# lrjconan/LanczosNetwork

Measured on AMD Instinct MI355X. Metric: molecules/sec LanczosNet forward, QM8 batch=1024, higher is better.
Workload: dtype f32; 1 GPU; QM8 LanczosNet batch=1024/GPU, N<=32 dense L (tile N=26), K=20, fp32, 7x128 layers, 1xMI355X per rank; step = [pack L + batch plan + Lanczos + tridiagonal eigensolver (Ritz pairs)] (one launch) + spectral gains + fused forward; global_batch=1024, parallelism=dp1 (batch shards, async score all-gather per step)

## Files before the change

lanczosnet_amd/csrc/gains_body.hpp:

```cpp
#pragma once
#include "common.hpp"

namespace lnz_gains {

constexpr int HID = 128;
constexpr int HT = HID / 32;
constexpr int SMAX = 16;
constexpr int OFF_W0 = 0;
constexpr int OFF_B0 = OFF_W0 + HT * 8 * 64;
constexpr int OFF_B2 = OFF_B0 + HT * 1024;
constexpr int OFF_B4 = OFF_B2 + HT * 1024;
constexpr int OFF_B6 = OFF_B4 + HT * 1024;
constexpr int OFF_W2 = OFF_B6 + 1024;
constexpr int OFF_W4 = OFF_W2 + HT * 16 * 256;
constexpr int OFF_W6 = OFF_W4 + HT * 16 * 256;
#ifndef LNZ_GAINS_RING
#define LNZ_GAINS_RING 8
#endif
#ifndef LNZ_GAINS_DIST
#define LNZ_GAINS_DIST (LNZ_GAINS_RING - 2)
#endif
constexpr int RING = LNZ_GAINS_RING;
constexpr int PACK_SIZE = OFF_W6 + 16 * 256 + RING * 256;
constexpr int NSTEP = 2 * HT * 16 + 16;

struct DistArr {
  int32_t v[SMAX];
};

__device__ inline float powi(float x, int p) {
  double base = (double)x, acc = 1.0;
  int e = p < 0 ? -p : p;
  while (e) {
    if (e & 1) acc *= base;
    base *= base;
    e >>= 1;
  }
  return (float)(p < 0 ? 1.0 / acc : acc);
}

__device__ inline f32x16 load_bias_frag(const float* __restrict__ bp, int lane) {
  const float4* p = reinterpret_cast<const float4*>(bp) + lane * 4;
  f32x16 acc;
#pragma unroll
  for (int g = 0; g < 4; ++g) {
    float4 v = p[g];
    acc[4 * g + 0] = v.x;
    acc[4 * g + 1] = v.y;
    acc[4 * g + 2] = v.z;
    acc[4 * g + 3] = v.w;
  }
  return acc;
}

__device__ inline f32x16 relu_bias16(f32x16 v, f32x16 b) {
#pragma unroll
  for (int i = 0; i < 16; ++i) v[i] = fmaxf(v[i] + b[i], 0.0f);
  return v;
}

template <int F0, int RT>
__device__ inline void dense_tile(const float4* __restrict__ wstream, float4 (&ring)[RING],
                                  const f32x16 (&Hin)[RT][HT], f32x16 (&res)[RT]) {
  f32x16 acc[RT], acc1[RT];
#pragma unroll
  for (int t = 0; t < RT; ++t) {
    acc[t] = lnz::splat16(0.0f);
    acc1[t] = lnz::splat16(0.0f);
  }
#pragma unroll
  for (int q = 0; q < 16; ++q) {
    constexpr int D = LNZ_GAINS_DIST;
#ifdef LNZ_GAINS_PROBE_NOLOAD
    ring[(F0 + q + D) % RING] = make_float4(0.5f, 0.25f, 0.125f, 1.0f);
#else
    ring[(F0 + q + D) % RING] = wstream[(F0 + q + D) * 64];
#endif
    __builtin_amdgcn_sched_barrier(0);
    const float4 a = ring[(F0 + q) % RING];
    const int ti = q >> 2, g = q & 3;
#pragma unroll
    for (int t = 0; t < RT; ++t) acc[t] = lnz::mfma32(a.x, Hin[t][ti][4 * g + 0], acc[t]);
#pragma unroll
    for (int t = 0; t < RT; ++t) acc1[t] = lnz::mfma32(a.y, Hin[t][ti][4 * g + 1], acc1[t]);
#pragma unroll
    for (int t = 0; t < RT; ++t) acc[t] = lnz::mfma32(a.z, Hin[t][ti][4 * g + 2], acc[t]);
#pragma unroll
    for (int t = 0; t < RT; ++t) acc1[t] = lnz::mfma32(a.w, Hin[t][ti][4 * g + 3], acc1[t]);
    __builtin_amdgcn_sched_barrier(0);
  }
#pragma unroll
  for (int t = 0; t < RT; ++t) {
#pragma unroll
    for (int i = 0; i < 16; ++i) res[t][i] = acc[t][i] + acc1[t][i];
  }
}

template <int RT>
__device__ __forceinline__ void gains_mlp_tiles(const float* __restrict__ D, const int (&row)[RT],
                                                const bool (&valid)[RT], const int l,
                                                const int lane, int B, int K, const DistArr& dist,
                                                int S, const float* __restrict__ mlp_pack,
                                                float* __restrict__ G) {
  const int hh = lane >> 5;
  const float* pk = mlp_pack + (int64_t)l * PACK_SIZE;
#ifdef LNZ_GAINS_PROBE_STAGGER
  for (int i = 0; i < (int)((blockIdx.x & (LNZ_GAINS_PROBE_STAGGER_N - 1)) * LNZ_GAINS_PROBE_STAGGER); ++i)
    __builtin_amdgcn_s_sleep(16);
#endif

  const float4* __restrict__ wstream = reinterpret_cast<const float4*>(pk + OFF_W2) + lane;
  float4 ring[RING];
#pragma unroll
  for (int f = 0; f < LNZ_GAINS_DIST; ++f) ring[f] = wstream[f * 64];

  const int steps0 = S < 8 ? S : 8;
  f32x16 h1[RT][HT], h2[RT][HT];
  {
    float w0[HT][8];
#pragma unroll
    for (int ot = 0; ot < HT; ++ot) {
#pragma unroll
      for (int t = 0; t < 8; ++t) w0[ot][t] = pk[OFF_W0 + (ot * 8 + t) * 64 + lane];
    }
#pragma unroll
    for (int rt = 0; rt < RT; ++rt) {
      const float dval = valid[rt] ? D[row[rt]] : 0.0f;
      float feat[8];
#pragma unroll
      for (int t = 0; t < 8; ++t) {
#ifdef LNZ_GAINS_PROBE_NOPOW
        float lo = t < S ? dval : 0.0f;
        float hi = (8 + t) < S ? dval : 0.0f;
#else
        float lo = t < S ? powi(dval, dist.v[t]) : 0.0f;
        float hi = (8 + t) < S ? powi(dval, dist.v[8 + t]) : 0.0f;
#endif
        feat[t] = hh ? hi : lo;
      }
#pragma unroll
      for (int ot = 0; ot < HT; ++ot) {
        f32x16 acc = lnz::splat16(0.0f);
#pragma unroll
        for (int t = 0; t < 8; ++t) {
          if (t < steps0) acc = lnz::mfma32(w0[ot][t], feat[t], acc);
        }
        h1[rt][ot] = relu_bias16(acc, load_bias_frag(pk + OFF_B0 + ot * 1024, lane));
      }
    }
  }
  f32x16 res[RT];
#define LNZ_DENSE(F0, IN, OUT, OT, BOFF)                                   \
  {                                                                        \
    const f32x16 bb = load_bias_frag(pk + (BOFF), lane);                   \
    dense_tile<F0, RT>(wstream, ring, IN, res);                            \
    _Pragma("unroll") for (int rt = 0; rt < RT; ++rt) OUT[rt][OT] = relu_bias16(res[rt], bb); \
  }
  LNZ_DENSE(0, h1, h2, 0, OFF_B2 + 0 * 1024)
  LNZ_DENSE(16, h1, h2, 1, OFF_B2 + 1 * 1024)
  LNZ_DENSE(32, h1, h2, 2, OFF_B2 + 2 * 1024)
  LNZ_DENSE(48, h1, h2, 3, OFF_B2 + 3 * 1024)
  LNZ_DENSE(64, h2, h1, 0, OFF_B4 + 0 * 1024)
  LNZ_DENSE(80, h2, h1, 1, OFF_B4 + 1 * 1024)
  LNZ_DENSE(96, h2, h1, 2, OFF_B4 + 2 * 1024)
  LNZ_DENSE(112, h2, h1, 3, OFF_B4 + 3 * 1024)
#undef LNZ_DENSE
  {
    const f32x16 b6 = load_bias_frag(pk + OFF_B6, lane);
    dense_tile<128, RT>(wstream, ring, h1, res);
#pragma unroll
    for (int rt = 0; rt < RT; ++rt) {
      if (valid[rt]) {
        const int b = row[rt] / K, k = row[rt] - b * K;
        float* Gb = G + (((int64_t)l * B + b) * S) * K + k;
#pragma unroll
        for (int r = 0; r < 16; ++r) {
          int sidx = lnz::cd_row(r, hh);
          if (sidx < S) Gb[(int64_t)sidx * K] = res[rt][r] + b6[r];
        }
      }
    }
  }
}

__device__ __forceinline__ void gains_mlp_tile(const float* __restrict__ D, const int row,
                                               const bool valid, const int l, const int lane,
                                               int B, int K, const DistArr& dist, int S,
                                               const float* __restrict__ mlp_pack,
                                               float* __restrict__ G) {
  const int rows1[1] = {row};
  const bool valid1[1] = {valid};
  gains_mlp_tiles<1>(D, rows1, valid1, l, lane, B, K, dist, S, mlp_pack, G);
}

}
```

lanczosnet_amd/csrc/lanczos_ritz.hip:

```cpp
#include "common.hpp"
#include "prep.hpp"
#include "gains_body.hpp"

namespace {

constexpr double kBreakdownTol = 1e-8;
constexpr double kEps = 2.220446049250313e-16;

struct Ritz32Smem {
  static constexpr int LD = 34;
  double* Qt;
  double* za;
  double* zb;
  double* ca;
  double* cb;
  double* dd;
  double* Dw;
  double2* de;
  int* perm;
  float* sgn;
  int NR;
  __device__ __forceinline__ double& dw(int hh, int i, int rr) const { return Dw[(hh * NR + i) * 32 + rr]; }
};

// ... 729 lines not shown
      const bool on = r < kk;
      double v[16];
      load16(&sm.Qt[(on ? sm.perm[r] : 0) * LD + 16 * h], v);
      double best = 0.0;
      float sg = 1.0f;
#pragma unroll
      for (int x = 0; x < 16; ++x) {
        const double av = fabs(v[x]);
        const bool take = av > best;
        sg = take ? (v[x] < 0 ? -1.0f : 1.0f) : sg;
        best = take ? av : best;
      }
      double best_up;
      const double best_lo = both_halves(best, best_up);
      int sg_up;
      const int sg_lo = both_halves(__float_as_int(sg), sg_up);
      if (on && h == 0) sm.sgn[r] = __int_as_float(best_up > best_lo ? sg_up : sg_lo);
    }
    __syncthreads();
  }

  for (int k = lane; k < K; k += 64) D[(int64_t)b * K + k] = k < kk ? (float)sm.dd[sm.perm[k]] : 0.0f;
  float* Vb = V + (int64_t)b * N * K;
  if (K <= 64) {
    const int rpp = 64 / K;
    const int rr0 = lane / K, k = lane - rr0 * K;
    const bool lane_on = rr0 < rpp, col_on = lane_on && k < kk;
    const double* col = &sm.Qt[(col_on ? sm.perm[k] : 0) * LD];
    const float sg = col_on ? sm.sgn[k] : 0.0f;
#pragma unroll 4
    for (int r0 = 0; r0 < N; r0 += rpp) {
      const int rr = r0 + rr0;
      if (lane_on && rr < N) Vb[rr * K + k] = (col_on && rr < n) ? sg * (float)col[rr] : 0.0f;
    }
  } else {
    const int dq = 64 / K, dr = 64 - dq * K;
    int rr = lane / K, k = lane - rr * K;
    for (int idx = lane; idx < N * K; idx += 64) {
      float v = 0.0f;
      if (rr < n && k < kk) v = sm.sgn[k] * (float)sm.Qt[sm.perm[k] * LD + rr];
      Vb[idx] = v;
      rr += dq;
      k += dr;
      if (k >= K) k -= K, ++rr;
    }
  }
  if (info && lane == 0) info[b] = nrestart;
#ifdef LNZ_PROFILE_PHASES
  __syncthreads();
  if (lane == 0) {
    long long tp3 = clock64();
    D[(int64_t)b * K + 0] = (float)(tp1 - tp0);
    D[(int64_t)b * K + 1] = (float)(tp2 - tp1);
    D[(int64_t)b * K + 2] = (float)(tp3 - tp2);
    D[(int64_t)b * K + 3] = (float)n;
    D[(int64_t)b * K + 4] = (float)(tsx[1] - tsx[0]);
    D[(int64_t)b * K + 5] = (float)(tsx[2] - tsx[1]);
    D[(int64_t)b * K + 6] = (float)(tsx[3] - tsx[2]);
    D[(int64_t)b * K + 7] = (float)(tsx[4] - tsx[1]);
    D[(int64_t)b * K + 8] = (float)(tsx[5] - tsx[4]);
  }
#endif
}

#ifdef LNZ_RITZ_VGPR160
#define LNZ_RITZ32_ATTR __attribute__((amdgpu_num_vgpr(80)))
#else
#define LNZ_RITZ32_ATTR
#endif
__global__ __launch_bounds__(64) LNZ_RITZ32_ATTR void lanczos_ritz32_kernel(
    const float* __restrict__ A, int64_t sb, int64_t sr, int64_t sc,
    const int32_t* __restrict__ n_nodes, int N, int K, float* __restrict__ D,
    float* __restrict__ V, int32_t* __restrict__ info) {
  extern __shared__ __attribute__((aligned(16))) unsigned char ubuf[];
  lanczos_ritz32_body(A, sb, sr, sc, n_nodes, N, K, D, V, info, blockIdx.x, threadIdx.x,
                      ritz32_view(ubuf, N));
}

__global__ __launch_bounds__(256) __attribute__((amdgpu_waves_per_eu(3)))
void prepare_batch_union_kernel(
    const float* __restrict__ L, int64_t sb, int64_t sr, int64_t sc, int64_t sch, int N, int C,
    float4* __restrict__ Lp, const uint8_t* __restrict__ mask, int B, int n_cu, int allow_pairs,
    int wg_cap, int32_t* __restrict__ plan, int32_t* __restrict__ n_wg, int K,
    int32_t* __restrict__ gain_rows, int32_t* __restrict__ n_gain_rows,
    const int32_t* __restrict__ n_nodes, float* __restrict__ D, float* __restrict__ V,
    int32_t* __restrict__ info, uint32_t* __restrict__ ident, int32_t* __restrict__ strips,
    int32_t* __restrict__ n_strips) {
  extern __shared__ __attribute__((aligned(16))) unsigned char ubuf[];
  const int blk = blockIdx.x;
#ifdef LNZ_PREP_X_NOPLAN
  if (blk < 2) return;
#endif
#ifdef LNZ_PREP_X_EMPTYPACK
  if (blk > B + 1) return;
#endif
  if (blk < 2) {
    __builtin_amdgcn_s_setprio(3);
    if (blk == 0)
      plan_tiles_body(mask, B, N, n_cu, allow_pairs, wg_cap, plan, n_wg, K, gain_rows, n_gain_rows);
    else if (strips)
      plan_strips_body(mask, B, N, n_cu, strips, n_strips, ubuf);
  } else if (blk <= B + 1) {
    if (threadIdx.x >= 64) return;
    lanczos_ritz32_body(L, sb, sr, sc, n_nodes, N, K, D, V, info, blk - 2, threadIdx.x,
                        ritz32_view(ubuf, N));
  } else {
    pack_laplacian_body(L, sb, sr, sc, sch, N, C, Lp, reinterpret_cast<float*>(ubuf), blk - 2 - B,
                        ident);
  }
}

static size_t prep_lds_bytes(int N, int C) {
  size_t lds = (size_t)N * N * C * sizeof(float);
  lds = lds > ritz32_lds_bytes(N) ? lds : ritz32_lds_bytes(N);
  return lds > (size_t)kStripScratch ? lds : (size_t)kStripScratch;
}

__global__ __launch_bounds__(256, 2) void prepare_batch_gains_kernel(
    const float* __restrict__ L, int64_t sb, int64_t sr, int64_t sc, int64_t sch, int N, int C,
    float4* __restrict__ Lp, const uint8_t* __restrict__ mask, int B, int n_cu, int allow_pairs,
    int wg_cap, int32_t* __restrict__ plan, int32_t* __restrict__ n_wg, int K,
    int32_t* __restrict__ gain_rows, int32_t* __restrict__ n_gain_rows,
    const int32_t* __restrict__ n_nodes, float* __restrict__ D, float* __restrict__ V,
    lnz_gains::DistArr dist, int S, int num_layer,
    const float* __restrict__ mlp_pack, float* __restrict__ G, uint32_t* __restrict__ ident,
    int n_cons, const float* __restrict__ Dg, const int32_t* __restrict__ rows_g,
    const int32_t* __restrict__ n_rows_g, int Bg, int32_t* __restrict__ strips,
    int32_t* __restrict__ n_strips) {
  extern __shared__ __attribute__((aligned(16))) unsigned char ubuf[];
  const Ritz32Smem sm = ritz32_view(ubuf, N);
  float* tile = reinterpret_cast<float*>(ubuf);
  const int blk = blockIdx.x;
  if (blk < 2) {
    __builtin_amdgcn_s_setprio(3);
    if (blk == 0)
      plan_tiles_body(mask, B, N, n_cu, allow_pairs, wg_cap, plan, n_wg, K, gain_rows, n_gain_rows);
    else if (strips)
      plan_strips_body(mask, B, N, n_cu, strips, n_strips, ubuf);
  } else if (blk <= B + 1) {
    if (threadIdx.x >= 64) return;
    __builtin_amdgcn_s_setprio(3);
    lanczos_ritz32_body(L, sb, sr, sc, n_nodes, N, K, D, V, nullptr, blk - 2, threadIdx.x, sm);
  } else {
    const int p = blk - B - 2;
    if (p >= n_cons) {
      pack_laplacian_body(L, sb, sr, sc, sch, N, C, Lp, tile, p - n_cons, ident);
      return;
    }
    const int lane = threadIdx.x & 63;
    const int gw = p * 4 + (threadIdx.x >> 6);
    const int t = gw / num_layer, l = gw - t * num_layer;
    const int R = *n_rows_g;
    if (32 * t >= R) return;
    const int idx = 32 * t + (lane & 31);
    const bool valid = idx < R;
    const int row = valid ? rows_g[idx] : 0;
    lnz_gains::gains_mlp_tile(Dg, row, valid, l, lane, Bg, K, dist, S, mlp_pack, G);
  }
}

}

extern "C" int lnz_prepare_batch(const float* L, int64_t stride_b, int64_t stride_r,
                                 int64_t stride_c, int64_t stride_ch, int B, int N, int C,
                                 float* Lp, const uint8_t* mask, const int32_t* n_nodes, int n_cu,
                                 int allow_pairs, int32_t* plan, int32_t* n_wg, int K,
                                 int32_t* gain_rows, int32_t* n_gain_rows, float* D, float* V,
                                 int32_t* info, uint32_t* ident, int32_t* strips,
                                 int32_t* n_strips, lnz_stream_t stream) {
  LNZ_REQUIRE(L && mask && n_nodes && plan && n_wg && D && V && B > 0 && C > 0 &&
                  C <= LNZ_MAX_CHANNELS && n_cu > 0 && K > 0,
              LNZ_EINVAL, "lnz_prepare_batch: bad arguments (B=%d C=%d K=%d)", B, C, K);
  LNZ_REQUIRE(Lp || !ident, LNZ_EINVAL, "lnz_prepare_batch: ident needs Lp (the pack writes both)");
  LNZ_REQUIRE(N > 0 && N <= LNZ_TILE, LNZ_ENOTSUP, "lnz_prepare_batch: N=%d > %d", N, LNZ_TILE);
  LNZ_REQUIRE(!gain_rows || n_gain_rows, LNZ_EINVAL, "lnz_prepare_batch: gain_rows needs n_gain_rows");
  const size_t tile = (size_t)N * N * C * sizeof(float);
  LNZ_REQUIRE(tile <= 40 * 1024, LNZ_ENOTSUP,
              "lnz_prepare_batch: N*N*C*4 = %zu B exceeds the 40 KiB staging tile", tile);
  LNZ_REQUIRE(!strips || n_strips, LNZ_EINVAL, "lnz_prepare_batch: strips need n_strips");
  hipLaunchKernelGGL(prepare_batch_union_kernel, dim3(Lp ? 2 * B + 2 : B + 2), dim3(256),
                     Lp ? prep_lds_bytes(N, C) : prep_lds_bytes(N, 0),
                     (hipStream_t)stream, L, stride_b, stride_r, stride_c, stride_ch, N, C,
                     (float4*)Lp, mask, B, n_cu, allow_pairs, lnz_plan_wg_cap(B, n_cu), plan, n_wg,
                     K, gain_rows, n_gain_rows, n_nodes, D, V, info, ident, strips, n_strips);
  return lnz::check_launch("lnz_prepare_batch");
}

extern "C" int lnz_prepare_batch_prev_gains(
    const float* L, int64_t stride_b, int64_t stride_r, int64_t stride_c, int64_t stride_ch, int B,
    int N, int C, float* Lp, const uint8_t* mask, const int32_t* n_nodes, int n_cu, int allow_pairs,
    int32_t* plan, int32_t* n_wg, int K, int32_t* gain_rows, int32_t* n_gain_rows, float* D,
    float* V, uint32_t* ident, const float* D_prev, int B_prev, const int32_t* rows_prev,
    const int32_t* n_rows_prev, const int32_t* dist_host, int S, int num_layer,
    const float* mlp_pack, float* G_prev, int32_t* strips, int32_t* n_strips,
    lnz_stream_t stream) {
  LNZ_REQUIRE(L && Lp && mask && n_nodes && plan && n_wg && gain_rows && n_gain_rows && D && V &&
                  D_prev && rows_prev && n_rows_prev && dist_host && mlp_pack && G_prev && B > 0 &&
                  B_prev > 0 && C > 0 && C <= LNZ_MAX_CHANNELS && n_cu > 0 && K > 0 && num_layer > 0,
              LNZ_EINVAL, "lnz_prepare_batch_prev_gains: bad arguments (B=%d C=%d K=%d)", B, C, K);
  LNZ_REQUIRE(N > 0 && N <= LNZ_TILE, LNZ_ENOTSUP, "lnz_prepare_batch_prev_gains: N=%d > %d", N,
              LNZ_TILE);
  LNZ_REQUIRE(S >= 1 && S <= lnz_gains::SMAX, LNZ_ENOTSUP, "lnz_prepare_batch_prev_gains: S=%d", S);
  const size_t tile = (size_t)N * N * C * sizeof(float);
  LNZ_REQUIRE(tile <= 40 * 1024, LNZ_ENOTSUP,
              "lnz_prepare_batch_prev_gains: N*N*C*4 = %zu B exceeds the 40 KiB staging tile", tile);
  lnz_gains::DistArr dist;
  for (int i = 0; i < lnz_gains::SMAX; ++i) dist.v[i] = i < S ? dist_host[i] : 0;
  const int64_t tiles = ((int64_t)B_prev * K + 31) / 32;
  const int64_t n_cons = (tiles * num_layer + 3) / 4;
  const int64_t grid = 2 * (int64_t)B + 2 + n_cons;
  LNZ_REQUIRE(grid < (1ll << 31), LNZ_ENOTSUP, "lnz_prepare_batch_prev_gains: batch too large");
  hipLaunchKernelGGL(prepare_batch_gains_kernel, dim3((unsigned)grid), dim3(256),
                     prep_lds_bytes(N, C), (hipStream_t)stream, L, stride_b, stride_r, stride_c, stride_ch, N, C,
                     (float4*)Lp, mask, B, n_cu, allow_pairs, lnz_plan_wg_cap(B, n_cu), plan, n_wg,
                     K, gain_rows, n_gain_rows, n_nodes, D, V, dist, S, num_layer, mlp_pack, G_prev,
                     ident, (int)n_cons, D_prev, rows_prev, n_rows_prev, B_prev,
                     (strips && n_strips) ? strips : nullptr, n_strips);
  return lnz::check_launch("lnz_prepare_batch_prev_gains");
}

int lnz_launch_ritz_wg(const float* A, int64_t stride_b, int64_t stride_r, int64_t stride_c,
                       const int32_t* n_nodes, int B, int N, int K, float* D, float* V,
                       int32_t* info, void* workspace, int64_t workspace_bytes, int flags,
                       hipStream_t s);

extern "C" int lnz_lanczos_ritz(const float* A, int64_t stride_b, int64_t stride_r,
                                int64_t stride_c, const int32_t* n_nodes, int B, int N, int K,
                                float* D, float* V, int32_t* info, lnz_stream_t stream) {
  LNZ_REQUIRE(A && n_nodes && D && V && B > 0 && N > 0 && K > 0, LNZ_EINVAL,
              "lnz_lanczos_ritz: bad arguments (B=%d N=%d K=%d)", B, N, K);
  hipStream_t s = (hipStream_t)stream;
  if (N > 32)
    return lnz_launch_ritz_wg(A, stride_b, stride_r, stride_c, n_nodes, B, N, K, D, V, info, nullptr,
                              0, 0, s);
  hipLaunchKernelGGL(lanczos_ritz32_kernel, dim3(B), dim3(64), ritz32_lds_bytes(N), s, A, stride_b,
                     stride_r, stride_c, n_nodes, N, K, D, V, info);
  return lnz::check_launch("lnz_lanczos_ritz");
}

namespace {
__global__ __launch_bounds__(64) void tridiag_eigh_kernel(const double* __restrict__ diag,
                                                          const double* __restrict__ offd, int M,
                                                          double* __restrict__ R,
                                                          double* __restrict__ Bm) {
  constexpr int NMAX = 64, LD = NMAX + 2;
  __shared__ double Qt[NMAX * LD];
  __shared__ double dd[NMAX], ee[NMAX];
  __shared__ int perm[NMAX];
  const int b = blockIdx.x, lane = threadIdx.x, n = M;
  for (int idx = lane; idx < NMAX * LD; idx += 64) {
    int i = idx / LD, r = idx - i * LD;
    Qt[idx] = (i == r) ? 1.0 : 0.0;
  }
  dd[lane] = lane < n ? diag[(int64_t)b * M + lane] : 0.0;
  ee[lane] = lane < n - 1 ? offd[(int64_t)b * (M - 1) + lane] : 0.0;
  __syncthreads();
  double f = 0.0, tst1 = 0.0;
  for (int l = 0; l < n; ++l) {
    tst1 = fmax(tst1, fabs(dd[l]) + fabs(ee[l]));
    int m = l;
    while (m < n - 1 && fabs(ee[m]) > kEps * tst1) ++m;
    if (m > l) {
      int iter = 0;
      double el;
      do {
        ++iter;
        double g = dd[l];
        el = ee[l];
        double p = (dd[l + 1] - g) / (2.0 * el);
        double rr = sqrt(p * p + 1.0);
        if (p < 0) rr = -rr;
        const double dl = el / (p + rr), dl1 = el * (p + rr), hh = g - dl;
        __syncthreads();
        if (lane == 0) {
          dd[l] = dl;
          dd[l + 1] = dl1;
        }
        if (lane >= l + 2 && lane < n) dd[lane] -= hh;
        __syncthreads();
        f += hh;
        p = dd[m];
        double c = 1.0, c2 = 1.0, c3 = 1.0, s = 0.0, s2 = 0.0;
        const double el1 = ee[l + 1];
        double carry = Qt[m * LD + lane];
        for (int i = m - 1; i >= l; --i) {
          c3 = c2;
          c2 = c;
          s2 = s;
          const double ei = ee[i], di = dd[i];
          g = c * ei;
          const double hp = c * p;
          const double tt = fma(p, p, ei * ei);
          const double rinv = rsqrt(tt), rad = tt * rinv;
          const double e_next = s * rad;
          s = ei * rinv;
          c = p * rinv;
          p = c * di - s * g;
          const double d_next = hp + s * (c * g + s * di);
          ee[i + 1] = e_next;
          dd[i + 1] = d_next;
          const double z0 = Qt[i * LD + lane];
          Qt[(i + 1) * LD + lane] = s * z0 + c * carry;
          carry = c * z0 - s * carry;
        }
        Qt[l * LD + lane] = carry;
        p = -s * s2 * c3 * el1 * ee[l] / dl1;
        el = s * p;
        __syncthreads();
        if (lane == 0) {
          ee[l] = el;
// ... 37 lines not shown
```

lanczosnet_amd/csrc/spectral_gains.hip:

```cpp
#include "common.hpp"
#include "gains_body.hpp"
#include "split_pack.hpp"
#include <stdlib.h>

namespace {

using namespace lnz_gains;

__global__ void pack_w0_kernel(const float* __restrict__ W0, int S, float* __restrict__ out) {
  int idx = blockIdx.x * blockDim.x + threadIdx.x;
  if (idx >= HT * 8 * 64) return;
  int lane = idx & 63, t = (idx >> 6) & 7, ot = idx >> 9;
  int f = 8 * (lane >> 5) + t;
  out[idx] = f < S ? W0[(32 * ot + (lane & 31)) * S + f] : 0.0f;
}

struct SplitRide {
  const float4* pack;
  float4* dst;
  int64_t n4;
  int main_x;
};
__device__ __forceinline__ bool ride_along(const SplitRide& r, const int lane) {
  if (!r.pack || (int)blockIdx.x < r.main_x) return false;
  const int64_t chunk = (int64_t)(blockIdx.x - r.main_x) * gridDim.y + blockIdx.y;
  if (chunk * lnz::kSplitChunk < r.n4) lnz::split_pack_chunk<64>(r.pack, r.dst, r.n4, chunk, lane);
  return true;
}

__global__ __launch_bounds__(64) void spectral_gains_mlp_kernel(
    const float* __restrict__ D, int R, int B, int K, DistArr dist, int S,
    const float* __restrict__ mlp_pack, const int32_t* __restrict__ rows,
    const int32_t* __restrict__ n_rows, float* __restrict__ G, const SplitRide ride) {
  const int lane = threadIdx.x;
  if (ride_along(ride, lane)) return;
  if (rows) R = *n_rows;
  if ((int)blockIdx.x * 32 >= R) return;
  const int idx = blockIdx.x * 32 + (lane & 31);
  const bool valid = idx < R;
  const int row = valid ? (rows ? rows[idx] : idx) : 0;
  gains_mlp_tile(D, row, valid, blockIdx.y, lane, B, K, dist, S, mlp_pack, G);
}

__global__ __launch_bounds__(64) void spectral_gains_mlp2_kernel(
    const float* __restrict__ D, int R, int B, int K, DistArr dist, int S,
    const float* __restrict__ mlp_pack, const int32_t* __restrict__ rows,
    const int32_t* __restrict__ n_rows, float* __restrict__ G, const SplitRide ride) {
  const int lane = threadIdx.x;
  if (ride_along(ride, lane)) return;
  if (rows) R = *n_rows;
  if ((int)blockIdx.x * 64 >= R) return;
  int row[2];
  bool valid[2];
#pragma unroll
  for (int t = 0; t < 2; ++t) {
    const int idx = blockIdx.x * 64 + 32 * t + (lane & 31);
    valid[t] = idx < R;
    row[t] = valid[t] ? (rows ? rows[idx] : idx) : 0;
  }
  gains_mlp_tiles<2>(D, row, valid, blockIdx.y, lane, B, K, dist, S, mlp_pack, G);
}

__global__ void spectral_gains_pow_kernel(const float* __restrict__ D, int B, int K, DistArr dist,
                                          int S, int num_layer, float* __restrict__ G) {
  int64_t idx = (int64_t)blockIdx.x * blockDim.x + threadIdx.x;
  int64_t total = (int64_t)num_layer * B * S * K;
  if (idx >= total) return;
  int k = (int)(idx % K);
  int s = (int)((idx / K) % S);
  int b = (int)((idx / ((int64_t)K * S)) % B);
  G[idx] = powi(D[(int64_t)b * K + k], dist.v[s]);
}

}

extern "C" int64_t lnz_spectral_mlp_pack_size(int S) {
  (void)S;
  return PACK_SIZE;
}

extern "C" int lnz_pack_spectral_mlp(const float* W0, const float* b0, const float* W2,
                                     const float* b2, const float* W4, const float* b4,
                                     const float* W6, const float* b6, int S, float* pack,
                                     lnz_stream_t stream) {
  LNZ_REQUIRE(W0 && b0 && W2 && b2 && W4 && b4 && W6 && b6 && pack, LNZ_EINVAL,
              "lnz_pack_spectral_mlp: null pointer");
  LNZ_REQUIRE(S >= 1 && S <= SMAX, LNZ_ENOTSUP, "lnz_pack_spectral_mlp: S=%d not in 1..%d", S,
              SMAX);
  hipLaunchKernelGGL(pack_w0_kernel, dim3((HT * 8 * 64 + 255) / 256), dim3(256), 0,
                     (hipStream_t)stream, W0, S, pack + OFF_W0);
  int rc = lnz::check_launch("lnz_pack_spectral_mlp(W0)");
  if (rc) return rc;
  if ((rc = lnz_pack_bias_rows(b0, HID, pack + OFF_B0, stream))) return rc;
  if ((rc = lnz_pack_rows_k8(W2, HID, HID, HID, pack + OFF_W2, stream))) return rc;
  if ((rc = lnz_pack_bias_rows(b2, HID, pack + OFF_B2, stream))) return rc;
  if ((rc = lnz_pack_rows_k8(W4, HID, HID, HID, pack + OFF_W4, stream))) return rc;
  if ((rc = lnz_pack_bias_rows(b4, HID, pack + OFF_B4, stream))) return rc;
  if ((rc = lnz_pack_rows_k8(W6, S, HID, HID, pack + OFF_W6, stream))) return rc;
  if ((rc = lnz_pack_bias_rows(b6, S, pack + OFF_B6, stream))) return rc;
  return LNZ_OK;
}

struct MlpLayerPtrs {
  const float* p[16][8];
};

__device__ inline float rows_k8_elem(const float* __restrict__ W, int rows, int cols, int ld,
                                     int Q, int f) {
  const int idx4 = f >> 2, u = f & 3;
  const int lane = idx4 & 63, q = (idx4 >> 6) % Q, rt = (idx4 >> 6) / Q;
  const int row = 32 * rt + (lane & 31), col = 8 * q + 4 * (lane >> 5) + u;
  return (row < rows && col < cols) ? W[(int64_t)row * ld + col] : 0.0f;
}

__device__ inline float bias_rows_elem(const float* __restrict__ b, int rows, int f) {
  const int r = f & 15, lane = (f >> 4) & 63, rt = f >> 10;
  const int row = 32 * rt + lnz::cd_row(r, lane >> 5);
  return row < rows ? b[row] : 0.0f;
}

__global__ void pack_spectral_mlp_layers_kernel(MlpLayerPtrs ptrs, int S, float* __restrict__ pack) {
  const int f = blockIdx.x * blockDim.x + threadIdx.x;
  if (f >= PACK_SIZE) return;
  const int l = blockIdx.y;
  const float* const* pl = ptrs.p[l];
  float v = 0.0f;
  if (f < OFF_B0) {
    const int lane = f & 63, t = (f >> 6) & 7, ot = f >> 9;
    const int feat = 8 * (lane >> 5) + t;
    v = feat < S ? pl[0][(32 * ot + (lane & 31)) * S + feat] : 0.0f;
  } else if (f < OFF_B2) {
    v = bias_rows_elem(pl[1], HID, f - OFF_B0);
  } else if (f < OFF_B4) {
    v = bias_rows_elem(pl[3], HID, f - OFF_B2);
  } else if (f < OFF_B6) {
    v = bias_rows_elem(pl[5], HID, f - OFF_B4);
  } else if (f < OFF_W2) {
    v = bias_rows_elem(pl[7], S, f - OFF_B6);
  } else if (f < OFF_W4) {
    v = rows_k8_elem(pl[2], HID, HID, HID, HID / 8, f - OFF_W2);
  } else if (f < OFF_W6) {
    v = rows_k8_elem(pl[4], HID, HID, HID, HID / 8, f - OFF_W4);
  } else if (f < OFF_W6 + 16 * 256) {
    v = rows_k8_elem(pl[6], S, HID, HID, HID / 8, f - OFF_W6);
  }
  pack[(int64_t)l * PACK_SIZE + f] = v;
}

extern "C" int lnz_pack_spectral_mlp_layers(const float* const* ptrs, int num_layer, int S,
                                            float* pack, lnz_stream_t stream) {
  LNZ_REQUIRE(ptrs && pack && num_layer >= 1 && num_layer <= 16, LNZ_EINVAL,
              "lnz_pack_spectral_mlp_layers: bad arguments (L=%d)", num_layer);
  LNZ_REQUIRE(S >= 1 && S <= SMAX, LNZ_ENOTSUP, "lnz_pack_spectral_mlp_layers: S=%d not in 1..%d",
              S, SMAX);
  MlpLayerPtrs mp;
  for (int l = 0; l < 16; ++l)
    for (int i = 0; i < 8; ++i) {
      mp.p[l][i] = l < num_layer ? ptrs[l * 8 + i] : nullptr;
      LNZ_REQUIRE(l >= num_layer || mp.p[l][i], LNZ_EINVAL,
                  "lnz_pack_spectral_mlp_layers: null pointer (layer %d, tensor %d)", l, i);
    }
  hipLaunchKernelGGL(pack_spectral_mlp_layers_kernel, dim3((PACK_SIZE + 255) / 256, num_layer),
                     dim3(256), 0, (hipStream_t)stream, mp, S, pack);
  return lnz::check_launch("lnz_pack_spectral_mlp_layers");
}

extern "C" int lnz_spectral_gains_rows_split_to(const float* D, int B, int K, const int32_t* dist_host,
                                                int S, int num_layer, int kind, const float* mlp_pack,
                                                const int32_t* rows, const int32_t* n_rows, float* G,
                                                const float* Lp_split, uint16_t* Lp_dst, int64_t lp_floats,
                                                lnz_stream_t stream) {
  LNZ_REQUIRE(!Lp_split == !Lp_dst, LNZ_EINVAL, "lnz_spectral_gains_rows_split_to: pack and destination come together");
  LNZ_REQUIRE(!rows || n_rows, LNZ_EINVAL, "lnz_spectral_gains_rows: rows without n_rows");
  LNZ_REQUIRE(!Lp_split || (kind == 0 && lp_floats > 0 && lp_floats % 4 == 0), LNZ_EINVAL,
              "lnz_spectral_gains_rows_split: the pack rides along with the MLP launch only (kind 0), "
              "lp_floats a positive multiple of 4");
  LNZ_REQUIRE(D && dist_host && G && B > 0 && K > 0 && num_layer > 0, LNZ_EINVAL,
              "lnz_spectral_gains: bad arguments (B=%d K=%d L=%d)", B, K, num_layer);
  LNZ_REQUIRE(S >= 1 && S <= SMAX, LNZ_ENOTSUP, "lnz_spectral_gains: S=%d not in 1..%d", S, SMAX);
  DistArr dist;
  for (int i = 0; i < SMAX; ++i) dist.v[i] = i < S ? dist_host[i] : 0;
  hipStream_t s = (hipStream_t)stream;
  if (kind == 0) {
    LNZ_REQUIRE(mlp_pack, LNZ_EINVAL, "lnz_spectral_gains: kind=MLP needs mlp_pack");
    int R = B * K;
    static const int forced = [] {
      const char* e = getenv("LNZ_GAINS_TILES");
      return e ? atoi(e) : 0;
    }();
    const bool two = forced ? forced == 2 : (int64_t)((R + 31) / 32) * num_layer >= 2048;
    SplitRide ride = {reinterpret_cast<const float4*>(Lp_split), reinterpret_cast<float4*>(Lp_dst), lp_floats / 4,
                      (R + (two ? 63 : 31)) / (two ? 64 : 32)};
    const int64_t chunks = Lp_split ? (ride.n4 + lnz::kSplitChunk - 1) / lnz::kSplitChunk : 0;
    const int64_t extra_x = (chunks + num_layer - 1) / num_layer;
    LNZ_REQUIRE(ride.main_x + extra_x < (1ll << 31), LNZ_ENOTSUP, "lnz_spectral_gains_rows_split: pack too large");
    dim3 grid((unsigned)(ride.main_x + extra_x), num_layer);
    if (two) {
      hipLaunchKernelGGL(spectral_gains_mlp2_kernel, grid, dim3(64), 0, s, D, R, B, K, dist, S,
                         mlp_pack, rows, n_rows, G, ride);
    } else {
      hipLaunchKernelGGL(spectral_gains_mlp_kernel, grid, dim3(64), 0, s, D, R, B, K, dist, S,
                         mlp_pack, rows, n_rows, G, ride);
    }
  } else {
    int64_t total = (int64_t)num_layer * B * S * K;
    hipLaunchKernelGGL(spectral_gains_pow_kernel, dim3((int)((total + 255) / 256)), dim3(256), 0,
                       s, D, B, K, dist, S, num_layer, G);
  }
  return lnz::check_launch("lnz_spectral_gains");
}

extern "C" int lnz_spectral_gains_rows_split(const float* D, int B, int K, const int32_t* dist_host,
                                             int S, int num_layer, int kind, const float* mlp_pack,
                                             const int32_t* rows, const int32_t* n_rows, float* G,
                                             float* Lp_split, int64_t lp_floats, lnz_stream_t stream) {
  return lnz_spectral_gains_rows_split_to(D, B, K, dist_host, S, num_layer, kind, mlp_pack, rows, n_rows, G,
                                          Lp_split, reinterpret_cast<uint16_t*>(Lp_split), lp_floats, stream);
}

extern "C" int lnz_spectral_gains_rows(const float* D, int B, int K, const int32_t* dist_host,
                                       int S, int num_layer, int kind, const float* mlp_pack,
                                       const int32_t* rows, const int32_t* n_rows, float* G,
                                       lnz_stream_t stream) {
  return lnz_spectral_gains_rows_split_to(D, B, K, dist_host, S, num_layer, kind, mlp_pack, rows, n_rows, G,
                                          nullptr, nullptr, 0, stream);
}

extern "C" int lnz_spectral_gains(const float* D, int B, int K, const int32_t* dist_host, int S,
                                  int num_layer, int kind, const float* mlp_pack, float* G,
                                  lnz_stream_t stream) {
  return lnz_spectral_gains_rows(D, B, K, dist_host, S, num_layer, kind, mlp_pack, nullptr,
                                 nullptr, G, stream);
}
```

Before: 1.349 million molecules/s.

## Rewrite spectral gains MLP with 16x16 MFMA tiles and persistent grid

Switches the per-row spectral-gains MLP from 32x32x2 MFMA tiles to 16x16x4 MFMA tiles. Each step now streams weights and biases from a single interleaved pack with a permuted feature order, so K-dimension waste for small S shrinks and the bias fragment loads disappear. The gains launch becomes a persistent grid sized to 8 waves per CU that walks (layer, tile) units in pairs, and the split-pack copy is folded into the same waves. It also changes the fused Ritz kernel's call site. This risks register pressure and more MFMA issue count per row, and the load balance now depends on the CU-count query.

```diff
diff --git a/lanczosnet_amd/csrc/gains_body.hpp b/lanczosnet_amd/csrc/gains_body.hpp
--- a/lanczosnet_amd/csrc/gains_body.hpp
+++ b/lanczosnet_amd/csrc/gains_body.hpp
@@ -4,16 +4,15 @@
 namespace lnz_gains {
 
 constexpr int HID = 128;
-constexpr int HT = HID / 32;
+constexpr int MT = HID / 16;
 constexpr int SMAX = 16;
-constexpr int OFF_W0 = 0;
-constexpr int OFF_B0 = OFF_W0 + HT * 8 * 64;
-constexpr int OFF_B2 = OFF_B0 + HT * 1024;
-constexpr int OFF_B4 = OFF_B2 + HT * 1024;
-constexpr int OFF_B6 = OFF_B4 + HT * 1024;
-constexpr int OFF_W2 = OFF_B6 + 1024;
-constexpr int OFF_W4 = OFF_W2 + HT * 16 * 256;
-constexpr int OFF_W6 = OFF_W4 + HT * 16 * 256;
+
+constexpr int ST_L1 = 0;
+constexpr int ST_L2 = ST_L1 + 2 * MT;
+constexpr int ST_L3 = ST_L2 + 9 * MT;
+constexpr int ST_L4 = ST_L3 + 9 * MT;
+constexpr int NSTEP = ST_L4 + 9;
+constexpr int PACK_SIZE = NSTEP * 256;
 #ifndef LNZ_GAINS_RING
 #define LNZ_GAINS_RING 8
 #endif
@@ -21,12 +20,21 @@
 #define LNZ_GAINS_DIST (LNZ_GAINS_RING - 2)
 #endif
 constexpr int RING = LNZ_GAINS_RING;
-constexpr int PACK_SIZE = OFF_W6 + 16 * 256 + RING * 256;
-constexpr int NSTEP = 2 * HT * 16 + 16;
+constexpr int DIST = LNZ_GAINS_DIST;
 
 struct DistArr {
   int32_t v[SMAX];
 };
+
+__host__ __device__ inline int kord(int kk) { return ((kk & 1) << 2) | ((kk >> 1) << 1); }
+__host__ __device__ inline int feat_at(int p) {
+  const int r = p & 3;
+  return (p & ~15) + 8 * (r >> 1) + (r & 1) + kord((p >> 2) & 3);
+}
+__host__ __device__ inline int feat0(int s, int kk, int S) {
+  return S <= 8 ? 4 * s + kk : 2 * s + 8 * (kk & 1) + (kk >> 1);
+}
+__host__ __device__ inline int steps0(int S) { return S <= 8 ? (S + 3) / 4 : 4; }
 
 __device__ inline float powi(float x, int p) {
   double base = (double)x, acc = 1.0;
@@ -39,158 +47,141 @@
   return (float)(p < 0 ? 1.0 / acc : acc);
 }
 
-__device__ inline f32x16 load_bias_frag(const float* __restrict__ bp, int lane) {
-  const float4* p = reinterpret_cast<const float4*>(bp) + lane * 4;
-  f32x16 acc;
-#pragma unroll
-  for (int g = 0; g < 4; ++g) {
-    float4 v = p[g];
-    acc[4 * g + 0] = v.x;
-    acc[4 * g + 1] = v.y;
-    acc[4 * g + 2] = v.z;
-    acc[4 * g + 3] = v.w;
-  }
-  return acc;
+__device__ __forceinline__ f32x4 mfma16(float a, float b, f32x4 c) {
+  return __builtin_amdgcn_mfma_f32_16x16x4f32(a, b, c, 0, 0, 0);
 }
 
-__device__ inline f32x16 relu_bias16(f32x16 v, f32x16 b) {
-#pragma unroll
-  for (int i = 0; i < 16; ++i) v[i] = fmaxf(v[i] + b[i], 0.0f);
+__device__ __forceinline__ float4 stream_step(const float4* __restrict__ ws, float4 (&ring)[RING],
+                                             const int F) {
+  if (F + DIST < NSTEP) ring[(F + DIST) % RING] = ws[(F + DIST) * 64];
+  __builtin_amdgcn_sched_barrier(0);
+  return ring[F % RING];
+}
+
+__device__ __forceinline__ f32x4 relu_bias4(f32x4 v, float4 b) {
+  v[0] = fmaxf(v[0] + b.x, 0.0f);
+  v[1] = fmaxf(v[1] + b.y, 0.0f);
+  v[2] = fmaxf(v[2] + b.z, 0.0f);
+  v[3] = fmaxf(v[3] + b.w, 0.0f);
   return v;
 }
 
-template <int F0, int RT>
-__device__ inline void dense_tile(const float4* __restrict__ wstream, float4 (&ring)[RING],
-                                  const f32x16 (&Hin)[RT][HT], f32x16 (&res)[RT]) {
-  f32x16 acc[RT], acc1[RT];
+template <int F, int NT, int NOUT, bool RELU>
+__device__ __forceinline__ void dense_layer(const float4* __restrict__ ws, float4 (&ring)[RING],
+                                            const f32x4 (&IN)[NT][MT], f32x4 (&OUT)[NT][MT]) {
 #pragma unroll
-  for (int t = 0; t < RT; ++t) {
-    acc[t] = lnz::splat16(0.0f);
-    acc1[t] = lnz::splat16(0.0f);
-  }
+  for (int mt = 0; mt < NOUT; ++mt) {
+    f32x4 acc0[NT], acc1[NT];
 #pragma unroll
-  for (int q = 0; q < 16; ++q) {
-    constexpr int D = LNZ_GAINS_DIST;
-#ifdef LNZ_GAINS_PROBE_NOLOAD
-    ring[(F0 + q + D) % RING] = make_float4(0.5f, 0.25f, 0.125f, 1.0f);
-#else
-    ring[(F0 + q + D) % RING] = wstream[(F0 + q + D) * 64];
-#endif
-    __builtin_amdgcn_sched_barrier(0);
-    const float4 a = ring[(F0 + q) % RING];
-    const int ti = q >> 2, g = q & 3;
+    for (int t = 0; t < NT; ++t) {
+      acc0[t] = f32x4{0.f, 0.f, 0.f, 0.f};
+      acc1[t] = f32x4{0.f, 0.f, 0.f, 0.f};
+    }
 #pragma unroll
-    for (int t = 0; t < RT; ++t) acc[t] = lnz::mfma32(a.x, Hin[t][ti][4 * g + 0], acc[t]);
+    for (int w = 0; w < 8; ++w) {
+      const float4 a = stream_step(ws, ring, F + 9 * mt + w);
 #pragma unroll
-    for (int t = 0; t < RT; ++t) acc1[t] = lnz::mfma32(a.y, Hin[t][ti][4 * g + 1], acc1[t]);
+      for (int t = 0; t < NT; ++t) acc0[t] = mfma16(a.x, IN[t][w][0], acc0[t]);
 #pragma unroll
-    for (int t = 0; t < RT; ++t) acc[t] = lnz::mfma32(a.z, Hin[t][ti][4 * g + 2], acc[t]);
+      for (int t = 0; t < NT; ++t) acc1[t] = mfma16(a.y, IN[t][w][1], acc1[t]);
 #pragma unroll
-    for (int t = 0; t < RT; ++t) acc1[t] = lnz::mfma32(a.w, Hin[t][ti][4 * g + 3], acc1[t]);
-    __builtin_amdgcn_sched_barrier(0);
-  }
+      for (int t = 0; t < NT; ++t) acc0[t] = mfma16(a.z, IN[t][w][2], acc0[t]);
 #pragma unroll
-  for (int t = 0; t < RT; ++t) {
+      for (int t = 0; t < NT; ++t) acc1[t] = mfma16(a.w, IN[t][w][3], acc1[t]);
+      __builtin_amdgcn_sched_barrier(0);
+    }
+    const float4 bb = stream_step(ws, ring, F + 9 * mt + 8);
 #pragma unroll
-    for (int i = 0; i < 16; ++i) res[t][i] = acc[t][i] + acc1[t][i];
+    for (int t = 0; t < NT; ++t) {
+      f32x4 v = acc0[t] + acc1[t];
+      if (RELU) {
+        v = relu_bias4(v, bb);
+      } else {
+        v[0] += bb.x;
+        v[1] += bb.y;
+        v[2] += bb.z;
+        v[3] += bb.w;
+      }
+      OUT[t][mt] = v;
+    }
   }
 }
 
-template <int RT>
-__device__ __forceinline__ void gains_mlp_tiles(const float* __restrict__ D, const int (&row)[RT],
-                                                const bool (&valid)[RT], const int l,
-                                                const int lane, int B, int K, const DistArr& dist,
-                                                int S, const float* __restrict__ mlp_pack,
-                                                float* __restrict__ G) {
-  const int hh = lane >> 5;
-  const float* pk = mlp_pack + (int64_t)l * PACK_SIZE;
-#ifdef LNZ_GAINS_PROBE_STAGGER
-  for (int i = 0; i < (int)((blockIdx.x & (LNZ_GAINS_PROBE_STAGGER_N - 1)) * LNZ_GAINS_PROBE_STAGGER); ++i)
-    __builtin_amdgcn_s_sleep(16);
-#endif
-
-  const float4* __restrict__ wstream = reinterpret_cast<const float4*>(pk + OFF_W2) + lane;
+template <int NT>
+__device__ __forceinline__ void gains_pass(const float* __restrict__ D, const int (&row)[NT],
+                                           const bool (&valid)[NT], const int l, const int lane,
+                                           int B, int K, const DistArr& dist, int S,
+                                           const float* __restrict__ mlp_pack,
+                                           float* __restrict__ G) {
+  const int kk = lane >> 4;
+  const float4* __restrict__ ws =
+      reinterpret_cast<const float4*>(mlp_pack + (int64_t)l * PACK_SIZE) + lane;
   float4 ring[RING];
 #pragma unroll
-  for (int f = 0; f < LNZ_GAINS_DIST; ++f) ring[f] = wstream[f * 64];
+  for (int f = 0; f < DIST; ++f) ring[f] = ws[f * 64];
 
-  const int steps0 = S < 8 ? S : 8;
-  f32x16 h1[RT][HT], h2[RT][HT];
-  {
-    float w0[HT][8];
+  int dv[SMAX];
 #pragma unroll
-    for (int ot = 0; ot < HT; ++ot) {
+  for (int i = 0; i < SMAX; ++i) dv[i] = __builtin_amdgcn_readfirstlane(dist.v[i]);
+  const int n1 = steps0(S);
+  float feat[NT][4];
 #pragma unroll
-      for (int t = 0; t < 8; ++t) w0[ot][t] = pk[OFF_W0 + (ot * 8 + t) * 64 + lane];
+  for (int s = 0; s < 4; ++s) {
+    const int f = feat0(s, kk, S);
+    int p;
+    if (S <= 8)
+      p = kk == 0 ? dv[4 * s] : kk == 1 ? dv[4 * s + 1] : kk == 2 ? dv[4 * s + 2] : dv[4 * s + 3];
+    else
+      p = kk == 0 ? dv[2 * s] : kk == 1 ? dv[2 * s + 8] : kk == 2 ? dv[2 * s + 1] : dv[2 * s + 9];
+#pragma unroll
+    for (int t = 0; t < NT; ++t) {
+      const float dval = valid[t] ? D[row[t]] : 0.0f;
+      feat[t][s] = f < S ? powi(dval, p) : 0.0f;
     }
+  }
+
+  f32x4 hA[NT][MT], hB[NT][MT];
 #pragma unroll
-    for (int rt = 0; rt < RT; ++rt) {
-      const float dval = valid[rt] ? D[row[rt]] : 0.0f;
-      float feat[8];
+  for (int mt = 0; mt < MT; ++mt) {
+    const float4 a = stream_step(ws, ring, ST_L1 + 2 * mt);
+    const float av[4] = {a.x, a.y, a.z, a.w};
+    f32x4 acc[NT];
 #pragma unroll
-      for (int t = 0; t < 8; ++t) {
-#ifdef LNZ_GAINS_PROBE_NOPOW
-        float lo = t < S ? dval : 0.0f;
-        float hi = (8 + t) < S ? dval : 0.0f;
-#else
-        float lo = t < S ? powi(dval, dist.v[t]) : 0.0f;
-        float hi = (8 + t) < S ? powi(dval, dist.v[8 + t]) : 0.0f;
-#endif
-        feat[t] = hh ? hi : lo;
-      }
+    for (int t = 0; t < NT; ++t) acc[t] = f32x4{0.f, 0.f, 0.f, 0.f};
 #pragma unroll
-      for (int ot = 0; ot < HT; ++ot) {
-        f32x16 acc = lnz::splat16(0.0f);
+    for (int s = 0; s < 4; ++s) {
+      if (s < n1) {
 #pragma unroll
-        for (int t = 0; t < 8; ++t) {
-          if (t < steps0) acc = lnz::mfma32(w0[ot][t], feat[t], acc);
-        }
-        h1[rt][ot] = relu_bias16(acc, load_bias_frag(pk + OFF_B0 + ot * 1024, lane));
+        for (int t = 0; t < NT; ++t) acc[t] = mfma16(av[s], feat[t][s], acc[t]);
       }
     }
+    __builtin_amdgcn_sched_barrier(0);
+    const float4 bb = stream_step(ws, ring, ST_L1 + 2 * mt + 1);
+#pragma unroll
+    for (int t = 0; t < NT; ++t) hA[t][mt] = relu_bias4(acc[t], bb);
   }
-  f32x16 res[RT];
-#define LNZ_DENSE(F0, IN, OUT, OT, BOFF)                                   \
-  {                                                                        \
-    const f32x16 bb = load_bias_frag(pk + (BOFF), lane);                   \
-    dense_tile<F0, RT>(wstream, ring, IN, res);                            \
-    _Pragma("unroll") for (int rt = 0; rt < RT; ++rt) OUT[rt][OT] = relu_bias16(res[rt], bb); \
-  }
-  LNZ_DENSE(0, h1, h2, 0, OFF_B2 + 0 * 1024)
-  LNZ_DENSE(16, h1, h2, 1, OFF_B2 + 1 * 1024)
-  LNZ_DENSE(32, h1, h2, 2, OFF_B2 + 2 * 1024)
-  LNZ_DENSE(48, h1, h2, 3, OFF_B2 + 3 * 1024)
-  LNZ_DENSE(64, h2, h1, 0, OFF_B4 + 0 * 1024)
-  LNZ_DENSE(80, h2, h1, 1, OFF_B4 + 1 * 1024)
-  LNZ_DENSE(96, h2, h1, 2, OFF_B4 + 2 * 1024)
-  LNZ_DENSE(112, h2, h1, 3, OFF_B4 + 3 * 1024)
-#undef LNZ_DENSE
-  {
-    const f32x16 b6 = load_bias_frag(pk + OFF_B6, lane);
-    dense_tile<128, RT>(wstream, ring, h1, res);
+  dense_layer<ST_L2, NT, MT, true>(ws, ring, hA, hB);
+  dense_layer<ST_L3, NT, MT, true>(ws, ring, hB, hA);
+  dense_layer<ST_L4, NT, 1, false>(ws, ring, hA, hB);
 #pragma unroll
-    for (int rt = 0; rt < RT; ++rt) {
-      if (valid[rt]) {
-        const int b = row[rt] / K, k = row[rt] - b * K;
-        float* Gb = G + (((int64_t)l * B + b) * S) * K + k;
+  for (int t = 0; t < NT; ++t) {
+    if (valid[t]) {
+      const int b = row[t] / K, k = row[t] - b * K;
+      float* Gb = G + (((int64_t)l * B + b) * S) * K + k;
 #pragma unroll
-        for (int r = 0; r < 16; ++r) {
-          int sidx = lnz::cd_row(r, hh);
-          if (sidx < S) Gb[(int64_t)sidx * K] = res[rt][r] + b6[r];
-        }
+      for (int r = 0; r < 4; ++r) {
+        const int sidx = 4 * kk + r;
+        if (sidx < S) Gb[(int64_t)sidx * K] = hB[t][0][r];
       }
     }
   }
 }
 
-__device__ __forceinline__ void gains_mlp_tile(const float* __restrict__ D, const int row,
-                                               const bool valid, const int l, const int lane,
-                                               int B, int K, const DistArr& dist, int S,
-                                               const float* __restrict__ mlp_pack,
-                                               float* __restrict__ G) {
-  const int rows1[1] = {row};
-  const bool valid1[1] = {valid};
-  gains_mlp_tiles<1>(D, rows1, valid1, l, lane, B, K, dist, S, mlp_pack, G);
+__device__ __forceinline__ void tile_row(const int32_t* __restrict__ rows, int R, int64_t tile,
+                                         int lane, int& row, bool& valid) {
+  const int64_t idx = 16 * tile + (lane & 15);
+  valid = idx < R;
+  row = valid ? (rows ? rows[idx] : (int)idx) : 0;
 }
 
 }
diff --git a/lanczosnet_amd/csrc/lanczos_ritz.hip b/lanczosnet_amd/csrc/lanczos_ritz.hip
--- a/lanczosnet_amd/csrc/lanczos_ritz.hip
+++ b/lanczosnet_amd/csrc/lanczos_ritz.hip
@@ -905,10 +905,11 @@
     const int t = gw / num_layer, l = gw - t * num_layer;
     const int R = *n_rows_g;
     if (32 * t >= R) return;
-    const int idx = 32 * t + (lane & 31);
-    const bool valid = idx < R;
-    const int row = valid ? rows_g[idx] : 0;
-    lnz_gains::gains_mlp_tile(Dg, row, valid, l, lane, Bg, K, dist, S, mlp_pack, G);
+    int row[2];
+    bool valid[2];
+    lnz_gains::tile_row(rows_g, R, 2 * t, lane, row[0], valid[0]);
+    lnz_gains::tile_row(rows_g, R, 2 * t + 1, lane, row[1], valid[1]);
+    lnz_gains::gains_pass<2>(Dg, row, valid, l, lane, Bg, K, dist, S, mlp_pack, G);
   }
 }
 
diff --git a/lanczosnet_amd/csrc/spectral_gains.hip b/lanczosnet_amd/csrc/spectral_gains.hip
--- a/lanczosnet_amd/csrc/spectral_gains.hip
+++ b/lanczosnet_amd/csrc/spectral_gains.hip
@@ -1,64 +1,51 @@
 #include "common.hpp"
 #include "gains_body.hpp"
 #include "split_pack.hpp"
-#include <stdlib.h>
 
 namespace {
 
 using namespace lnz_gains;
 
-__global__ void pack_w0_kernel(const float* __restrict__ W0, int S, float* __restrict__ out) {
-  int idx = blockIdx.x * blockDim.x + threadIdx.x;
-  if (idx >= HT * 8 * 64) return;
-  int lane = idx & 63, t = (idx >> 6) & 7, ot = idx >> 9;
-  int f = 8 * (lane >> 5) + t;
-  out[idx] = f < S ? W0[(32 * ot + (lane & 31)) * S + f] : 0.0f;
-}
-
 struct SplitRide {
   const float4* pack;
   float4* dst;
   int64_t n4;
-  int main_x;
 };
-__device__ __forceinline__ bool ride_along(const SplitRide& r, const int lane) {
-  if (!r.pack || (int)blockIdx.x < r.main_x) return false;
-  const int64_t chunk = (int64_t)(blockIdx.x - r.main_x) * gridDim.y + blockIdx.y;
-  if (chunk * lnz::kSplitChunk < r.n4) lnz::split_pack_chunk<64>(r.pack, r.dst, r.n4, chunk, lane);
-  return true;
-}
 
-__global__ __launch_bounds__(64) void spectral_gains_mlp_kernel(
-    const float* __restrict__ D, int R, int B, int K, DistArr dist, int S,
+__global__ __launch_bounds__(64) __attribute__((amdgpu_waves_per_eu(2))) void spectral_gains_kernel(
+    const float* __restrict__ D, int R, int B, int K, DistArr dist, int S, int num_layer,
     const float* __restrict__ mlp_pack, const int32_t* __restrict__ rows,
     const int32_t* __restrict__ n_rows, float* __restrict__ G, const SplitRide ride) {
   const int lane = threadIdx.x;
-  if (ride_along(ride, lane)) return;
   if (rows) R = *n_rows;
-  if ((int)blockIdx.x * 32 >= R) return;
-  const int idx = blockIdx.x * 32 + (lane & 31);
-  const bool valid = idx < R;
-  const int row = valid ? (rows ? rows[idx] : idx) : 0;
-  gains_mlp_tile(D, row, valid, blockIdx.y, lane, B, K, dist, S, mlp_pack, G);
-}
-
-__global__ __launch_bounds__(64) void spectral_gains_mlp2_kernel(
-    const float* __restrict__ D, int R, int B, int K, DistArr dist, int S,
-    const float* __restrict__ mlp_pack, const int32_t* __restrict__ rows,
-    const int32_t* __restrict__ n_rows, float* __restrict__ G, const SplitRide ride) {
-  const int lane = threadIdx.x;
-  if (ride_along(ride, lane)) return;
-  if (rows) R = *n_rows;
-  if ((int)blockIdx.x * 64 >= R) return;
-  int row[2];
-  bool valid[2];
-#pragma unroll
-  for (int t = 0; t < 2; ++t) {
-    const int idx = blockIdx.x * 64 + 32 * t + (lane & 31);
-    valid[t] = idx < R;
-    row[t] = valid[t] ? (rows ? rows[idx] : idx) : 0;
+  const int64_t tl = (R + 15) / 16;
+  const int64_t T = tl * num_layer;
+  const int64_t W = gridDim.x, w = blockIdx.x;
+  int64_t u = T * w / W;
+  const int64_t end = T * (w + 1) / W;
+  while (u < end) {
+    const int l = (int)(u / tl);
+    const int64_t t = u - l * tl;
+    const int64_t left = end - u < tl - t ? end - u : tl - t;
+    if (left >= 2) {
+      int row[2];
+      bool valid[2];
+      tile_row(rows, R, t, lane, row[0], valid[0]);
+      tile_row(rows, R, t + 1, lane, row[1], valid[1]);
+      gains_pass<2>(D, row, valid, l, lane, B, K, dist, S, mlp_pack, G);
+      u += 2;
+    } else {
+      int row[1];
+      bool valid[1];
+      tile_row(rows, R, t, lane, row[0], valid[0]);
+      gains_pass<1>(D, row, valid, l, lane, B, K, dist, S, mlp_pack, G);
+      u += 1;
+    }
   }
-  gains_mlp_tiles<2>(D, row, valid, blockIdx.y, lane, B, K, dist, S, mlp_pack, G);
+  if (ride.pack) {
+    for (int64_t chunk = w; chunk * lnz::kSplitChunk < ride.n4; chunk += W)
+      lnz::split_pack_chunk<64>(ride.pack, ride.dst, ride.n4, chunk, lane);
+  }
 }
 
 __global__ void spectral_gains_pow_kernel(const float* __restrict__ D, int B, int K, DistArr dist,
@@ -79,72 +66,41 @@
   return PACK_SIZE;
 }
 
-extern "C" int lnz_pack_spectral_mlp(const float* W0, const float* b0, const float* W2,
-                                     const float* b2, const float* W4, const float* b4,
-                                     const float* W6, const float* b6, int S, float* pack,
-                                     lnz_stream_t stream) {
-  LNZ_REQUIRE(W0 && b0 && W2 && b2 && W4 && b4 && W6 && b6 && pack, LNZ_EINVAL,
-              "lnz_pack_spectral_mlp: null pointer");
-  LNZ_REQUIRE(S >= 1 && S <= SMAX, LNZ_ENOTSUP, "lnz_pack_spectral_mlp: S=%d not in 1..%d", S,
-              SMAX);
-  hipLaunchKernelGGL(pack_w0_kernel, dim3((HT * 8 * 64 + 255) / 256), dim3(256), 0,
-                     (hipStream_t)stream, W0, S, pack + OFF_W0);
-  int rc = lnz::check_launch("lnz_pack_spectral_mlp(W0)");
-  if (rc) return rc;
-  if ((rc = lnz_pack_bias_rows(b0, HID, pack + OFF_B0, stream))) return rc;
-  if ((rc = lnz_pack_rows_k8(W2, HID, HID, HID, pack + OFF_W2, stream))) return rc;
-  if ((rc = lnz_pack_bias_rows(b2, HID, pack + OFF_B2, stream))) return rc;
-  if ((rc = lnz_pack_rows_k8(W4, HID, HID, HID, pack + OFF_W4, stream))) return rc;
-  if ((rc = lnz_pack_bias_rows(b4, HID, pack + OFF_B4, stream))) return rc;
-  if ((rc = lnz_pack_rows_k8(W6, S, HID, HID, pack + OFF_W6, stream))) return rc;
-  if ((rc = lnz_pack_bias_rows(b6, S, pack + OFF_B6, stream))) return rc;
-  return LNZ_OK;
-}
-
 struct MlpLayerPtrs {
   const float* p[16][8];
 };
 
-__device__ inline float rows_k8_elem(const float* __restrict__ W, int rows, int cols, int ld,
-                                     int Q, int f) {
-  const int idx4 = f >> 2, u = f & 3;
-  const int lane = idx4 & 63, q = (idx4 >> 6) % Q, rt = (idx4 >> 6) / Q;
-  const int row = 32 * rt + (lane & 31), col = 8 * q + 4 * (lane >> 5) + u;
-  return (row < rows && col < cols) ? W[(int64_t)row * ld + col] : 0.0f;
-}
-
-__device__ inline float bias_rows_elem(const float* __restrict__ b, int rows, int f) {
-  const int r = f & 15, lane = (f >> 4) & 63, rt = f >> 10;
-  const int row = 32 * rt + lnz::cd_row(r, lane >> 5);
-  return row < rows ? b[row] : 0.0f;
-}
-
 __global__ void pack_spectral_mlp_layers_kernel(MlpLayerPtrs ptrs, int S, float* __restrict__ pack) {
   const int f = blockIdx.x * blockDim.x + threadIdx.x;
   if (f >= PACK_SIZE) return;
-  const int l = blockIdx.y;
-  const float* const* pl = ptrs.p[l];
+  const float* const* pl = ptrs.p[blockIdx.y];
+  const int step = f >> 8, lane = (f >> 2) & 63, u = f & 3;
+  const int kk = lane >> 4, i = lane & 15;
   float v = 0.0f;
-  if (f < OFF_B0) {
-    const int lane = f & 63, t = (f >> 6) & 7, ot = f >> 9;
-    const int feat = 8 * (lane >> 5) + t;
-    v = feat < S ? pl[0][(32 * ot + (lane & 31)) * S + feat] : 0.0f;
-  } else if (f < OFF_B2) {
-    v = bias_rows_elem(pl[1], HID, f - OFF_B0);
-  } else if (f < OFF_B4) {
-    v = bias_rows_elem(pl[3], HID, f - OFF_B2);
-  } else if (f < OFF_B6) {
-    v = bias_rows_elem(pl[5], HID, f - OFF_B4);
-  } else if (f < OFF_W2) {
-    v = bias_rows_elem(pl[7], S, f - OFF_B6);
-  } else if (f < OFF_W4) {
-    v = rows_k8_elem(pl[2], HID, HID, HID, HID / 8, f - OFF_W2);
-  } else if (f < OFF_W6) {
-    v = rows_k8_elem(pl[4], HID, HID, HID, HID / 8, f - OFF_W4);
-  } else if (f < OFF_W6 + 16 * 256) {
-    v = rows_k8_elem(pl[6], S, HID, HID, HID / 8, f - OFF_W6);
+  if (step < ST_L2) {
+    const int mt = step >> 1;
+    if (!(step & 1)) {
+      const int feat = feat0(u, kk, S);
+      if (u < steps0(S) && feat < S) v = pl[0][feat_at(16 * mt + i) * S + feat];
+    } else {
+      v = pl[1][feat_at(16 * mt + 4 * kk + u)];
+    }
+  } else {
+    const int layer = step < ST_L3 ? 1 : step < ST_L4 ? 2 : 3;
+    const int j = step - (layer == 1 ? ST_L2 : layer == 2 ? ST_L3 : ST_L4);
+    const int mt = j / 9, w = j % 9;
+    const float* W = pl[2 * layer];
+    const float* bias = pl[2 * layer + 1];
+    const int out = layer == 3 ? i : feat_at(16 * mt + i);
+    const int bout = layer == 3 ? 4 * kk + u : feat_at(16 * mt + 4 * kk + u);
+    const int nout = layer == 3 ? S : HID;
+    if (w < 8) {
+      if (out < nout) v = W[out * HID + feat_at(16 * w + 4 * kk + u)];
+    } else {
+      if (bout < nout) v = bias[bout];
+    }
   }
-  pack[(int64_t)l * PACK_SIZE + f] = v;
+  pack[(int64_t)blockIdx.y * PACK_SIZE + f] = v;
 }
 
 extern "C" int lnz_pack_spectral_mlp_layers(const float* const* ptrs, int num_layer, int S,
@@ -165,6 +121,24 @@
   return lnz::check_launch("lnz_pack_spectral_mlp_layers");
 }
 
+extern "C" int lnz_pack_spectral_mlp(const float* W0, const float* b0, const float* W2,
+                                     const float* b2, const float* W4, const float* b4,
+                                     const float* W6, const float* b6, int S, float* pack,
+                                     lnz_stream_t stream) {
+  LNZ_REQUIRE(W0 && b0 && W2 && b2 && W4 && b4 && W6 && b6 && pack, LNZ_EINVAL,
+              "lnz_pack_spectral_mlp: null pointer");
+  const float* ptrs[8] = {W0, b0, W2, b2, W4, b4, W6, b6};
+  return lnz_pack_spectral_mlp_layers(ptrs, 1, S, pack, stream);
+}
+
+static int gains_slots() {
+  int dev = 0, n_cu = 0;
+  if (hipGetDevice(&dev) != hipSuccess ||
+      hipDeviceGetAttribute(&n_cu, hipDeviceAttributeMultiprocessorCount, dev) != hipSuccess)
+    return 0;
+  return 8 * n_cu;
+}
+
 extern "C" int lnz_spectral_gains_rows_split_to(const float* D, int B, int K, const int32_t* dist_host,
                                                 int S, int num_layer, int kind, const float* mlp_pack,
                                                 const int32_t* rows, const int32_t* n_rows, float* G,
@@ -183,25 +157,15 @@
   hipStream_t s = (hipStream_t)stream;
   if (kind == 0) {
     LNZ_REQUIRE(mlp_pack, LNZ_EINVAL, "lnz_spectral_gains: kind=MLP needs mlp_pack");
-    int R = B * K;
-    static const int forced = [] {
-      const char* e = getenv("LNZ_GAINS_TILES");
-      return e ? atoi(e) : 0;
-    }();
-    const bool two = forced ? forced == 2 : (int64_t)((R + 31) / 32) * num_layer >= 2048;
-    SplitRide ride = {reinterpret_cast<const float4*>(Lp_split), reinterpret_cast<float4*>(Lp_dst), lp_floats / 4,
-                      (R + (two ? 63 : 31)) / (two ? 64 : 32)};
-    const int64_t chunks = Lp_split ? (ride.n4 + lnz::kSplitChunk - 1) / lnz::kSplitChunk : 0;
-    const int64_t extra_x = (chunks + num_layer - 1) / num_layer;
-    LNZ_REQUIRE(ride.main_x + extra_x < (1ll << 31), LNZ_ENOTSUP, "lnz_spectral_gains_rows_split: pack too large");
-    dim3 grid((unsigned)(ride.main_x + extra_x), num_layer);
-    if (two) {
-      hipLaunchKernelGGL(spectral_gains_mlp2_kernel, grid, dim3(64), 0, s, D, R, B, K, dist, S,
-                         mlp_pack, rows, n_rows, G, ride);
-    } else {
-      hipLaunchKernelGGL(spectral_gains_mlp_kernel, grid, dim3(64), 0, s, D, R, B, K, dist, S,
-                         mlp_pack, rows, n_rows, G, ride);
-    }
+    LNZ_REQUIRE((int64_t)B * K < (1ll << 31) - 16, LNZ_ENOTSUP, "lnz_spectral_gains: B*K too large");
+    const int R = B * K;
+    const int slots = gains_slots();
+    LNZ_REQUIRE(slots > 0, LNZ_ELAUNCH, "lnz_spectral_gains: no device");
+    const int64_t units = (int64_t)((R + 15) / 16) * num_layer;
+    const int grid = (int)(units < slots ? units : slots);
+    SplitRide ride = {reinterpret_cast<const float4*>(Lp_split), reinterpret_cast<float4*>(Lp_dst), lp_floats / 4};
+    hipLaunchKernelGGL(spectral_gains_kernel, dim3(grid), dim3(64), 0, s, D, R, B, K, dist, S,
+                       num_layer, mlp_pack, rows, n_rows, G, ride);
   } else {
     int64_t total = (int64_t)num_layer * B * S * K;
     hipLaunchKernelGGL(spectral_gains_pow_kernel, dim3((int)((total + 255) / 256)), dim3(256), 0,
```

Result: no change. 1.347 million molecules/s, median of 3 (-0.1%).
